# stemangiola/ppcseq

Hardware: AMD Instinct MI355X
Metric: effective samples/sec (whole node) for NB hierarchical fit (higher is better)
Workload: dtype f64; 1 GPU; BASELINE cfg3: synthetic 20000 genes x 200 samples (seed 20253), C=2, K=1000; NUTS (Stan defaults) warm-up 150 + 250 kept draws/chain, 8 chains per GPU (cfg3 names 8 chains; chains are the sharded unit, so N GPUs run 8N chains); mode=chains, chains_total=8, lanes_per_gene=4, loglik_workgroups=939, ess_estimator=rank-normalised split-chain bulk-ESS, min over 6 hyper-parameters and lp__, grad_evals=1471121, divergent_after_warmup=0, round_structure=pipelined: merged log-likelihood / state-machine launch + gene kernel, stream_groups=library default (3 from eight chains on, 2 from four), rounds_last_step_all_groups=115040

## Files before the change

ppcseq_amd/csrc/ppcx_gene.h:

```cpp
#pragma once
#include "ppcx_nuts.h"


namespace ppcx {

template <int CM>
struct GeneCtx {
  static constexpr int NCM = CM + 1;
  int gg, ncoord;
  bool active, has_slopes, fast, two;
  int idx[NCM];
  double q[NCM];
  GeneParams<CM> gp;
};

PPCX_HD void coord_consts(const Dims& d, const VecRef& v, int i, double q) {
  if (i >= d.off_sigma_raw && i < d.off_tail) {
    v.at(V_C0, i) = fast_exp(-q); v.at(V_C2, i) = q;
  } else if (i >= d.off_intercept && i < d.off_sigma_raw) {
    v.at(V_C0, i) = fast_exp(q);
    if (d.raw_consts) v.at(V_C2, i) = q;
  }
}

template <int CM>
PPCX_HD void gene_index(const Dims& d, int g, GeneCtx<CM>& x) {
  constexpr int NCM = CM + 1;
  x.active = g < d.G;
  x.gg = x.active ? g : 0;
  const int C = d.C;
  const int nslope = x.gg < d.K ? (C - 1 > 1 ? C - 1 : 1) : 0;
  x.ncoord = x.active ? 2 + nslope : 0;
#pragma unroll
  for (int j = 0; j < NCM; ++j)
    x.idx[j] = j == 0 ? d.off_intercept + x.gg : (j == 1 ? d.off_sigma_raw + x.gg : coef_index(d, j - 1, x.gg));
  x.has_slopes = x.active && x.gg < d.K && C >= 2;
  x.two = x.has_slopes && d.x0_is_one && d.x1_binary;
  x.fast = d.x0_is_one && (!x.has_slopes || x.two);
}
template <int CM>
PPCX_HD void gene_params(const Dims& d, const VecRef& v, GeneCtx<CM>& x) {
  x.gp.coef[0] = x.q[0];
#pragma unroll
  for (int cc = 1; cc < CM; ++cc) x.gp.coef[cc] = (x.has_slopes && cc < d.C) ? x.q[cc + 1] : 0.0;
  x.gp.sigma_raw = x.q[1];
  x.gp.phi = x.active ? v.at(V_C0, x.idx[1]) : 1.0;
  x.gp.invphi = 0.0;
}
template <int CM>
PPCX_HD void gene_load(const Dims& d, const Cmd& c, const VecRef& v, int g, GeneCtx<CM>& x) {
  constexpr int NCM = CM + 1;
  gene_index<CM>(d, g, x);
#pragma unroll
  for (int j = 0; j < NCM; ++j) x.q[j] = j < x.ncoord ? v.at(V_Q0 + 3 * c.dir, x.idx[j]) : 0.0;
  gene_params<CM>(d, v, x);
}

struct CellData {
  const int* counts;
  const double* disp;
  const unsigned char* gflags;
  const double* Sy;
  const double* ncell;
  double e_min, e_max;
};

struct GenePre { double phi, sigma, a0, Sy, n; int flags; };
PPCX_HD GenePre gene_pre_load(const Dims& d, const VecRef& v, const CellData& m, int g) {
  GenePre r;
  r.phi = v.at(V_C0, d.off_sigma_raw + g);
  r.sigma = v.at(V_C2, d.off_sigma_raw + g);
  r.a0 = v.at(V_C0, d.off_intercept + g);
  r.Sy = m.Sy[g]; r.n = m.ncell[g]; r.flags = m.gflags[g];
  return r;
}
template <int L> struct DispDeal {
  static constexpr int NL = L >= 8 ? 4 : (L >= 4 ? 2 : 1);
  static constexpr int CH = kDispStride / NL;
};

template <int CM, int L, int MODE, bool MASKED, bool WIN>
PPCX_HD void sweep_cells(int S, const int* row, const double* sE, const double* sX1, int sub, double A, double A1, double one,
                         const GeneParams<CM>& gp, const double* tab, CellAcc<CM>& acc, const double* ec = nullptr, int C = 2) {
  const int nmin = S / L;
  const int nlane = nmin + (sub < S - nmin * L ? 1 : 0);
  const int* p = row + sub;
  const double* q = sE + sub;
  const double* qx = sX1 + sub;
  int y0 = p[0], y1 = p[L], y2 = p[2 * L], y3 = p[3 * L];
  int k = 0;
#define PPCX_SWEEP_CELL(Y, E, XB, OFF, COND)                                                    \
  if ((COND) && (!MASKED || (Y) >= 0)) {                                                        \
    if (MODE == 1) { const double a1_ = (XB) != 0.0 ? A1 : A;                                   \
                     const double rho_ = WIN ? cell_eval_win<CM, true>(Y, E, a1_, one, gp, tab, acc) : cell_eval<CM, true>(Y, E, a1_, gp, tab, acc); \
                     acc.Tx[1] = fma(XB, rho_, acc.Tx[1]); }                                    \
    else if (MODE == 2) {                                                                       \
      double a_ = (XB) != 0.0 ? A1 : A; double xk_[CM];                                         \
      _Pragma("unroll") for (int cc = 2; cc < CM; ++cc) { xk_[cc] = cc < C ? qx[(cc - 1) * S + (OFF)] : 0.0; a_ = xk_[cc] != 0.0 ? a_ * ec[cc] : a_; } \
      const double rho_ = WIN ? cell_eval_win<CM, true>(Y, E, a_, one, gp, tab, acc) : cell_eval<CM, true>(Y, E, a_, gp, tab, acc); \
      acc.Tx[1] = fma(XB, rho_, acc.Tx[1]);                                                     \
      _Pragma("unroll") for (int cc = 2; cc < CM; ++cc) acc.Tx[cc] = fma(xk_[cc], rho_, acc.Tx[cc]); \
    }                                                                                           \
    else if (MODE == 3) {                                                                       \
      double t_ = (XB) * ec[1]; double xk_[CM];                                                 \
      _Pragma("unroll") for (int cc = 2; cc < CM; ++cc) { xk_[cc] = cc < C ? qx[(cc - 1) * S + (OFF)] : 0.0; t_ = fma(xk_[cc], ec[cc], t_); } \
      const double rho_ = cell_eval<CM, true>(Y, E, A * fast_exp(t_), gp, tab, acc);           \
      acc.Tx[1] = fma(XB, rho_, acc.Tx[1]);                                                     \
      _Pragma("unroll") for (int cc = 2; cc < CM; ++cc) acc.Tx[cc] = fma(xk_[cc], rho_, acc.Tx[cc]); \
    }                                                                                           \
    else if (WIN) (void)cell_eval_win<CM, false>(Y, E, A, one, gp, tab, acc);                   \
    else (void)cell_eval<CM, false>(Y, E, A, gp, tab, acc);                                     \
  }
  for (; k + 4 <= nmin; k += 4) {
    const double e0 = q[0], e1 = q[L], e2 = q[2 * L], e3 = q[3 * L];
    double x0 = 0.0, x1 = 0.0, x2 = 0.0, x3 = 0.0;
    if (MODE != 0) { x0 = qx[0]; x1 = qx[L]; x2 = qx[2 * L]; x3 = qx[3 * L]; }
    p += 4 * L; q += 4 * L; qx += 4 * L;
    const int n0 = p[0], n1 = p[L], n2 = p[2 * L], n3 = p[3 * L];
    if (MODE == 0 && !MASKED && WIN) {
      CellMidWin c0, c1, c2, c3;
      (void)cell_front_win<CM, false>(y0, e0, A, one, gp, tab, acc, c0);
      (void)cell_front_win<CM, false>(y1, e1, A, one, gp, tab, acc, c1);
      (void)cell_front_win<CM, false>(y2, e2, A, one, gp, tab, acc, c2);
      (void)cell_front_win<CM, false>(y3, e3, A, one, gp, tab, acc, c3);
#if defined(__HIP_DEVICE_COMPILE__)
      __builtin_amdgcn_sched_barrier(0);
#endif
      cell_back_win<CM>(c0, acc); cell_back_win<CM>(c1, acc); cell_back_win<CM>(c2, acc); cell_back_win<CM>(c3, acc);
    } else if (MODE == 0 && !MASKED) {
      CellMid c0, c1, c2, c3;
      (void)cell_front<CM, false>(y0, e0, A, gp, tab, acc, c0);
      (void)cell_front<CM, false>(y1, e1, A, gp, tab, acc, c1);
      (void)cell_front<CM, false>(y2, e2, A, gp, tab, acc, c2);
      (void)cell_front<CM, false>(y3, e3, A, gp, tab, acc, c3);
#if defined(__HIP_DEVICE_COMPILE__)
      __builtin_amdgcn_sched_barrier(0);
#endif
      cell_back<CM>(c0, acc); cell_back<CM>(c1, acc); cell_back<CM>(c2, acc); cell_back<CM>(c3, acc);
    } else {
      PPCX_SWEEP_CELL(y0, e0, x0, -4 * L, true)
      PPCX_SWEEP_CELL(y1, e1, x1, -3 * L, true)
      PPCX_SWEEP_CELL(y2, e2, x2, -2 * L, true)
      PPCX_SWEEP_CELL(y3, e3, x3, -L, true)
    }
    y0 = n0; y1 = n1; y2 = n2; y3 = n3;
  }
  if (k < nlane) {
    const double e0 = q[0], e1 = q[L], e2 = q[2 * L], e3 = q[3 * L];
    double x0 = 0.0, x1 = 0.0, x2 = 0.0, x3 = 0.0;
    if (MODE != 0) { x0 = qx[0]; x1 = qx[L]; x2 = qx[2 * L]; x3 = qx[3 * L]; }
    PPCX_SWEEP_CELL(y0, e0, x0, 0, true)
    PPCX_SWEEP_CELL(y1, e1, x1, L, k + 1 < nlane)
    PPCX_SWEEP_CELL(y2, e2, x2, 2 * L, k + 2 < nlane)
    PPCX_SWEEP_CELL(y3, e3, x3, 3 * L, k + 3 < nlane)
  }
#undef PPCX_SWEEP_CELL
}

template <int CM, int L>
PPCX_HD void generic_cells(const Dims& d, const Cmd& c, const VecRef& v, int g, bool has_slopes, const int* row,
                           const double* sExpo, const double* sX, int sub, GeneParams<CM>& gp, const double* tab,
                           CellAcc<CM>& acc) {
  const int S = d.S, C = d.C;
  gp.coef[0] = v.at(V_C2, d.off_intercept + g);
#pragma unroll
  for (int cc = 1; cc < CM; ++cc) gp.coef[cc] = (has_slopes && cc < C) ? v.at(V_C2, coef_index(d, cc, g)) : 0.0;
  (void)c;
  for (int s = sub; s < S; s += L) {
    const int y = row[s];
    if (y >= 0) {
      double t = sExpo[s] + gp.sigma_raw;
#pragma unroll
      for (int cc = 0; cc < CM; ++cc) if (cc < C) t += sX[cc * S + s] * gp.coef[cc];
      const double u = fast_exp(t);
      const double rho = cell_eval<CM, true>(y, u, 1.0, gp, tab, acc);
#pragma unroll
      for (int cc = 0; cc < CM; ++cc) if (cc < C) acc.Tx[cc] = fma(sX[cc * S + s], rho, acc.Tx[cc]);
    }
  }
}

template <int CM, int L, int GEN = 3>
PPCX_HD void lane_gene_sums(const Dims& d, const Cmd& c, const VecRef& v, const CellData& m, int g, const GenePre& pre, int sub,
                            const double* sE, const double* sExpo, const double* sX, const double* tab, const double* wtab,
                            GeneSumsV<CM>& o
#ifdef PPCX_TRACE
                            , unsigned long long* trace_stamps = nullptr
#endif
                            ) {
#if defined(PPCX_TRACE) && defined(__HIP_DEVICE_COMPILE__)
#define PPCX_GSTAMP(k) do { if (trace_stamps) trace_stamps[k] = __builtin_readcyclecounter(); } while (0)
#else
#define PPCX_GSTAMP(k) ((void)0)
#endif
  const int S = d.S;
  const bool has_slopes = g < d.K && d.C >= 2;
  const bool two = has_slopes && d.x0_is_one && d.x1_binary;
  const bool lin = (GEN & 1) && d.x0_is_one && has_slopes && !two;
  const bool generic = (GEN & 2) && !d.x0_is_one;
  GeneParams<CM> gp;
  gp.phi = pre.phi;
  const double sigma = pre.sigma;
  gp.sigma_raw = sigma;
  gp.invphi = fast_rcp(gp.phi);
  const double A = pre.a0 * gp.invphi;
  const bool masked = (pre.flags & 1) != 0;
  const int* row = m.counts + (long)g * S;
  constexpr int NL = DispDeal<L>::NL, CH = DispDeal<L>::CH;
  const DispRef dr = disp_ref(sigma);
  const int fn = L == 1 ? 0 : sub / NL, jch = L == 1 ? 0 : sub - fn * NL;
  const bool tab_lane = dr.in && (L == 1 || fn < 2);
  const double* pc = m.disp + (((long)g * kDispPanels + dr.panel) * 2 + (fn & 1)) * kDispStride + jch * CH;
  double cf[CH], cf2[L == 1 ? CH : 1];
#pragma unroll
  for (int k = 0; k < CH; ++k) cf[k] = 0.0;
  cf2[0] = 0.0;
  if (tab_lane) {
#pragma unroll
    for (int k = 0; k < CH; ++k) cf[k] = pc[k];
    if (L == 1) {
#pragma unroll
      for (int k = 0; k < CH; ++k) cf2[k] = pc[kDispStride + k];
    }
  }
  CellAcc<CM> acc; acc.zero();
  PPCX_GSTAMP(5);
  if (GEN & 2) {
    if (PPCX_WAVE_ANY(generic)) {
      if (generic) generic_cells<CM, L>(d, c, v, g, has_slopes, row, sExpo, sX, sub, gp, tab, acc);
    }
  }
  GeneWindow gw; gw.k = 0; gw.ok = false; gw.scale = 1.0;
  bool win = false;
  if (!(GEN & 2) || PPCX_WAVE_ANY(!generic)) {
    if (!generic) {
      const bool any_masked = PPCX_WAVE_ANY(masked);
#define PPCX_SWEEP(MODE, A_LO, A_HI, A_, A1_, X1_, ...)                                                                  \
      gw = gene_window(fma(m.e_min, A_LO, 1.0), fma(m.e_max, A_HI, 1.0));                                                 \
      win = !any_masked && PPCX_WAVE_ALL(gw.ok);                                                                          \
      if (any_masked) sweep_cells<CM, L, MODE, true, false>(S, row, sE, X1_, sub, A_, A1_, 1.0, gp, tab, acc, ##__VA_ARGS__);   \
      else if (win) sweep_cells<CM, L, MODE, false, true>(S, row, sE, X1_, sub, (A_) * gw.scale, (A1_) * gw.scale, gw.scale, gp, wtab, acc, ##__VA_ARGS__); \
      else sweep_cells<CM, L, MODE, false, false>(S, row, sE, X1_, sub, A_, A1_, 1.0, gp, tab, acc, ##__VA_ARGS__);
      if ((GEN & 1) && PPCX_WAVE_ANY(lin)) {
        double be[CM];
        be[0] = 0.0;
#pragma unroll
        for (int cc = 1; cc < CM; ++cc) be[cc] = (lin && cc < d.C) ? v.at(V_C2, coef_index(d, cc, g)) : 0.0;
        if (any_masked) sweep_cells<CM, L, 3, true, false>(S, row, sE, sX + S, sub, A, A, 1.0, gp, tab, acc, be, d.C);
        else sweep_cells<CM, L, 3, false, false>(S, row, sE, sX + S, sub, A, A, 1.0, gp, tab, acc, be, d.C);
      } else if (CM > 2 && d.C > 2 && PPCX_WAVE_ANY(two)) {
        double ec[CM];
        ec[0] = 1.0;
        double a_lo = A, a_hi = A;
#pragma unroll
        for (int cc = 1; cc < CM; ++cc) {
          ec[cc] = (two && cc < d.C) ? v.at(V_C0, coef_index(d, cc, g)) : 1.0;
          a_lo = ec[cc] < 1.0 ? a_lo * ec[cc] : a_lo; a_hi = ec[cc] > 1.0 ? a_hi * ec[cc] : a_hi;
        }
        const double A1 = A * ec[1];
        PPCX_SWEEP(2, a_lo, a_hi, A, A1, sX + S, ec, d.C)
      } else if (PPCX_WAVE_ANY(two)) {
        const double A1 = two ? A * v.at(V_C0, coef_index(d, 1, g)) : A;
        PPCX_SWEEP(1, (A1 < A ? A1 : A), (A1 > A ? A1 : A), A, A1, sX + S)
      } else {
        PPCX_SWEEP(0, A, A, A, A, sX)
      }
#undef PPCX_SWEEP
    }
  }
  PPCX_GSTAMP(6);
  if (!win) gw.scale = 1.0;
  cell_acc_close<CM>(gp, acc, gw.scale, &o);
  if ((GEN & 1) && lin) o.Tx[0] = o.Sr;
  if (win && sub == 0 && gw.k != 0) {
    const double kd = (double)gw.k;
    const double klog2 = fma(kd, 6.93147180369123816490e-01, kd * 1.90821492927058770002e-10);
    o.lik -= klog2 * fma(gp.phi, pre.n, pre.Sy);
    o.dph -= klog2 * pre.n;
  }
  if (tab_lane) {
    double hv = cf[CH - 1];
#pragma unroll
    for (int k = CH - 2; k >= 0; --k) hv = fma(hv, dr.x, cf[k]);
    if (NL > 1) {
      const double x3 = dr.x * dr.x * dr.x, xc = CH == 3 ? x3 : x3 * x3;
      double xp = (jch & 1) ? xc : 1.0;
      if (NL > 2) xp = (jch & 2) ? xp * (xc * xc) : xp;
      hv *= xp;
    }
    if (L == 1) {
      double h2 = cf2[CH - 1];
#pragma unroll
      for (int k = CH - 2; k >= 0; --k) h2 = fma(h2, dr.x, cf2[k]);
      o.lik += hv; o.dph += h2;
    } else if (fn == 0) o.lik += hv;
    else o.dph += hv;
  }
  if (PPCX_WAVE_ANY(!dr.in)) {
    PPCX_KEEP_BRANCH();
    if (!dr.in) {
      double F, D;
      disp_row_at(row, S, sub, L, sigma, &F, &D);
      o.lik += F; o.dph += D;
    }
  }
}

struct GeneData { double Sy, SyE, ncell, Lg1, SyX[kMaxC], SX[kMaxC]; };
// ... 306 lines not shown
```

ppcseq_amd/csrc/ppcx_kernels.hip:

```cpp
#include <hip/hip_runtime.h>
#include <hip/hip_ext.h>
#include "ppcx_gene.h"
#include "ppcx_kernels.h"

namespace ppcx {

typedef int __attribute__((may_alias)) word_t;
typedef double2 __attribute__((may_alias)) dpair_t;

#ifndef PPCX_LOGLIK_OCC
#define PPCX_LOGLIK_OCC 2
#endif
#ifndef PPCX_LOGLIK_OCC_FAST
#define PPCX_LOGLIK_OCC_FAST 4
#endif
__device__ __forceinline__ double wave_xor_add_rt(double v, int lane_xor_mask) {
  const int src = (int)((threadIdx.x ^ (unsigned)lane_xor_mask) & 63u) << 2;
  const int lo = __builtin_amdgcn_ds_bpermute(src, __double2loint(v));
  const int hi = __builtin_amdgcn_ds_bpermute(src, __double2hiint(v));
  return v + __hiloint2double(hi, lo);
}
template <int CTRL, int ROW_MASK>
__device__ __forceinline__ double dpp_take(double v) {
  const int lo = __builtin_amdgcn_update_dpp(0, __double2loint(v), CTRL, ROW_MASK, 0xf, true);
  const int hi = __builtin_amdgcn_update_dpp(0, __double2hiint(v), CTRL, ROW_MASK, 0xf, true);
  return __hiloint2double(hi, lo);
}
template <int L>
__device__ __forceinline__ double group_sum(double v) {
  if (L >= 2) v += dpp_take<0xB1, 0xf>(v);
  if (L >= 4) v += dpp_take<0x4E, 0xf>(v);
  if (L >= 8) v += dpp_take<0x141, 0xf>(v);
  if (L >= 16) v += dpp_take<0x140, 0xf>(v);
  if (L >= 32) v = wave_xor_add_rt(v, 16);
  if (L >= 64) v = wave_xor_add_rt(v, 32);
  return v;
}
template <int CM, int LG, int GEN>
__device__ __forceinline__ void loglik_passes(const LoglikArgs& a, const Cmd& c, const VecRef& v, double* sums, int p0, int p1,
                                              const double* stab, const double* swin, const double* sE, const double* sExpo, const double* sX,
                                              int lane, bool any_generic) {
  constexpr int L = 1 << LG, GPW = 64 >> LG;
  const Dims& d = a.d;
  const int sub = lane & (L - 1), gl = lane >> LG;
  int g_cur = a.order[p0 + gl < p1 ? p0 + gl : p1 - 1];
  int g_next = a.order[p0 + GPW + gl < p1 ? p0 + GPW + gl : p1 - 1];
  GenePre pre_cur = gene_pre_load(d, v, a.cd, g_cur);
#ifdef PPCX_TRACE
  unsigned long long* tr = nullptr;
  if (a.trace && lane == 0 && (blockIdx.x % 16) == 0 && blockIdx.x / 16 < kTraceBlocks)
    tr = a.trace + (((long)(blockIdx.x / 16) * 4 + (threadIdx.x >> 6)) * kTracePasses) * kTraceStamps;
  int tpass = 0;
#define PPCX_STAMP(k) do { if (tr && tpass < kTracePasses) tr[tpass * kTraceStamps + (k)] = __builtin_readcyclecounter(); } while (0)
#else
#define PPCX_STAMP(k) ((void)0)
#endif
  for (int p = p0; p < p1; p += GPW) {
    PPCX_STAMP(0);
#ifdef PPCX_TRACE
    if (tr && tpass < kTracePasses) tr[tpass * kTraceStamps + 7] = __builtin_amdgcn_s_memrealtime();
#endif
#ifdef PPCX_PRIO_BALANCE
    {
      const int rem = (p1 - p + GPW - 1) / GPW;
      if (rem >= 4) __builtin_amdgcn_s_setprio(3); else if (rem == 3) __builtin_amdgcn_s_setprio(2); else if (rem == 2) __builtin_amdgcn_s_setprio(1); else __builtin_amdgcn_s_setprio(0);
    }
#endif
    const bool act = p + gl < p1;
    const int g = g_cur;
    const GenePre pre = pre_cur;
    if (p + GPW < p1) {
      g_cur = g_next;
      pre_cur = gene_pre_load(d, v, a.cd, g_next);
      const int pn = p + 2 * GPW + gl;
      g_next = a.order[pn < p1 ? pn : p1 - 1];
    }
    if (CM > 2 && d.x0_is_one && !PPCX_WAVE_ANY(g < d.K)) {
      GeneSumsV<2> o2;
      lane_gene_sums<2, L, 0>(d, c, v, a.cd, g, pre, sub, sE, sExpo, sX, stab, swin, o2);
      o2.lik = group_sum<L>(o2.lik); o2.dph = group_sum<L>(o2.dph); o2.Sr = group_sum<L>(o2.Sr);
      if (act && sub == 0) { const long G = d.G; sums[0 * G + g] = o2.lik; sums[1 * G + g] = o2.dph; sums[2 * G + g] = o2.Sr; }
      continue;
    }
    GeneSumsV<CM> o;
    PPCX_STAMP(1);
#ifdef PPCX_TRACE
    lane_gene_sums<CM, L, GEN>(d, c, v, a.cd, g, pre, sub, sE, sExpo, sX, stab, swin, o, (tr && tpass < kTracePasses) ? tr + tpass * kTraceStamps : nullptr);
#else
    lane_gene_sums<CM, L, GEN>(d, c, v, a.cd, g, pre, sub, sE, sExpo, sX, stab, swin, o);
#endif
    PPCX_STAMP(2);
    const bool with_tx = any_generic && (!d.x0_is_one || PPCX_WAVE_ANY(g < d.K));
    o.lik = group_sum<L>(o.lik); o.dph = group_sum<L>(o.dph); o.Sr = group_sum<L>(o.Sr);
    PPCX_STAMP(3);
    if (with_tx) {
#pragma unroll
      for (int cc = 0; cc < CM; ++cc) if (cc < d.C) o.Tx[cc] = group_sum<L>(o.Tx[cc]);
    }
    if (act && sub == 0) {
      const long G = d.G;
      sums[0 * G + g] = o.lik; sums[1 * G + g] = o.dph; sums[2 * G + g] = o.Sr;
      if (with_tx) {
#pragma unroll
        for (int cc = 0; cc < CM; ++cc) if (cc < d.C) sums[(3 + cc) * G + g] = o.Tx[cc];
      }
    }
    PPCX_STAMP(4);
#ifdef PPCX_TRACE
    ++tpass;
#endif
  }
#undef PPCX_STAMP
}

template <int CM, int GEN, bool PIPE>
__device__ __forceinline__ void loglik_role(const LoglikArgs& a, int jb, int col, double* lds) {
  if (jb >= a.nbpc) return;
  constexpr int NS = GeneSums<CM>::N;
  const Dims& d = a.d;
  const int S = d.S, C = d.C;
  const int tid = threadIdx.x;
  const int wave = tid >> 6, lane = tid & 63;
  static_assert(2 * kLogTabSize == 2 * 256, "one 16-byte request per thread fills the table");
  const bool any_generic = !d.x0_is_one || (C >= 2 && d.K > 0);
  const bool evenS = (S & 1) == 0;
  const int p0 = a.bounds[jb * 4 + wave], p1 = a.bounds[jb * 4 + wave + 1];
  const double2 f_tab = reinterpret_cast<const dpair_t*>(a.logtab)[tid];
  static_assert(2 * kWinTabSize == 4 * 2 * 256, "four 16-byte requests per thread fill the window table");
  double2 f_win[4];
#pragma unroll
  for (int k = 0; k < 4; ++k) f_win[k] = reinterpret_cast<const dpair_t*>(a.wintab)[tid + 256 * k];
  double2 f_e = {0.0, 0.0};
  if (evenS) { if (tid < S / 2) f_e = reinterpret_cast<const dpair_t*>(a.sampleE)[tid]; }
  else if (tid < S) f_e.x = a.sampleE[tid];
  double f_x = 0.0;
  if (GEN != 2 && any_generic && tid < S) f_x = a.X[S + tid];
  const int chain = a.active ? a.active[col] : col;
  const Cmd& c = a.cmds[chain];
  if (c.type == CMD_DONE || c.type == CMD_FLUSH) return;
  if (PIPE) {
    if (c.evaluated && c.type != CMD_LEAF) return;
  }
  double* stab = lds;
  double* swin = lds + 2 * kLogTabSize;
  double* sE = swin + 2 * kWinTabSize;
  double* sExpo = GEN == 2 ? sE + S + kLdsPad : nullptr;
  double* sX = GEN == 2 ? sExpo + S : sE + kLdsPad;
  const VecRef v{a.vecs + (long)chain * V_COUNT * a.Dpad, a.Dpad};
  double* sums = a.sums + (long)chain * NS * d.G;
  reinterpret_cast<dpair_t*>(stab)[tid] = f_tab;
#pragma unroll
  for (int k = 0; k < 4; ++k) reinterpret_cast<dpair_t*>(swin)[tid + 256 * k] = f_win[k];
  if (evenS) {
    if (tid < S / 2) reinterpret_cast<dpair_t*>(sE)[tid] = f_e;
    for (int i = tid + 256; i < S / 2; i += 256) reinterpret_cast<dpair_t*>(sE)[i] = reinterpret_cast<const dpair_t*>(a.sampleE)[i];
  } else {
    if (tid < S) sE[tid] = f_e.x;
    for (int i = tid + 256; i < S; i += 256) sE[i] = a.sampleE[i];
  }
  if (any_generic) {
    if (GEN == 2) {
      for (int i = tid; i < S; i += 256) sExpo[i] = a.exposure[i];
      for (int i = tid; i < S * C; i += 256) sX[i] = a.X[i];
    } else {
      if (tid < S) sX[S + tid] = f_x;
      for (int i = tid + 256; i < S; i += 256) sX[S + i] = a.X[S + i];
      for (int i = 2 * S + tid; i < S * C; i += 256) sX[i] = a.X[i];
    }
  }
  __syncthreads();
  if (p0 >= p1) return;
  switch (a.lgL) {
    case 0: loglik_passes<CM, 0, GEN>(a, c, v, sums, p0, p1, stab, swin, sE, sExpo, sX, lane, any_generic); break;
    case 1: loglik_passes<CM, 1, GEN>(a, c, v, sums, p0, p1, stab, swin, sE, sExpo, sX, lane, any_generic); break;
    case 2: loglik_passes<CM, 2, GEN>(a, c, v, sums, p0, p1, stab, swin, sE, sExpo, sX, lane, any_generic); break;
    case 3: loglik_passes<CM, 3, GEN>(a, c, v, sums, p0, p1, stab, swin, sE, sExpo, sX, lane, any_generic); break;
    case 4: loglik_passes<CM, 4, GEN>(a, c, v, sums, p0, p1, stab, swin, sE, sExpo, sX, lane, any_generic); break;
    case 5: loglik_passes<CM, 5, GEN>(a, c, v, sums, p0, p1, stab, swin, sE, sExpo, sX, lane, any_generic); break;
    default: loglik_passes<CM, 6, GEN>(a, c, v, sums, p0, p1, stab, swin, sE, sExpo, sX, lane, any_generic); break;
  }
}

template <int CM, int GEN>
__global__ __launch_bounds__(256, GEN ? PPCX_LOGLIK_OCC : PPCX_LOGLIK_OCC_FAST) void ppcx_loglik_kernel(LoglikArgs a) {
  extern __shared__ double lds[];
  const int nch = a.nchains;
  const int lin = blockIdx.x, run = lin / (8 * nch), r = lin - run * (8 * nch);
  loglik_role<CM, GEN, false>(a, run * 8 + (r & 7), r >> 3, lds);
}

__device__ __forceinline__ double wave_sum_to_lane63(double v) {
  v += dpp_take<0x111, 0xf>(v);
  v += dpp_take<0x112, 0xf>(v);
  v += dpp_take<0x114, 0xf>(v);
  v += dpp_take<0x118, 0xf>(v);
  v += dpp_take<0x142, 0xa>(v);
  v += dpp_take<0x143, 0xc>(v);
  return v;
}
template <int N>
__device__ __forceinline__ void block_accumulate(double* vals, double* wacc, int wave, int lane) {
#pragma unroll
  for (int k = 0; k < N; ++k) vals[k] = wave_sum_to_lane63(vals[k]);
  if (lane == 63) {
#pragma unroll
    for (int k = 0; k < N; ++k) wacc[wave * PT_COUNT + k] = vals[k];
  }
}
struct ScanSums {
  static constexpr bool kLevel0WithLeaf = false;
  double* wacc; int wave, lane;
  __device__ __forceinline__ double* begin(int, double* own) {
#pragma unroll
    for (int k = 0; k < 6; ++k) own[k] = 0.0;
    return own;
  }
  __device__ __forceinline__ void end(int off, double* six) { block_accumulate<6>(six, wacc + off, wave, lane); }
};
__device__ __forceinline__ void slab_row_write(const Cmd& c, const double* wacc, double* slab, int tid, bool keep_t0) {
  const int np = parts_used(c);
  for (int k = tid; k < np; k += 256) {
    if (keep_t0 && k == PT_T0) continue;
    const bool used = k < 10 || (k >= PT_DOTS && k < PT_DOTS + 6 * c.n_merge) || (k >= PT_TOP && c.subtree_complete);
    slab[k] = used ? ((wacc[k] + wacc[PT_COUNT + k]) + wacc[2 * PT_COUNT + k]) + wacc[3 * PT_COUNT + k] : 0.0;
  }
}

constexpr int kRowStride = 65, kPartStride = 16, kRowsPerWave = 16;
template <int N>
__device__ __forceinline__ void wave_sums_lds(const double* vals, double* rows, double* out , int lane) {
  static_assert(N >= 1 && N <= kRowsPerWave, "one batch");
#pragma unroll
  for (int k = 0; k < N; ++k) rows[k * kRowStride + lane + (kPartStride - 16) * (lane >> 4)] = vals[k];
  __builtin_amdgcn_fence(__ATOMIC_RELEASE, "wavefront");
  __builtin_amdgcn_wave_barrier();
  const int k = lane >> 2, part = lane & 3;
  double t = 0.0;
  if (k < N) {
    const double* r = rows + k * kRowStride + kPartStride * part;
    double b[8];
#pragma unroll
    for (int j = 0; j < 8; ++j) b[j] = r[2 * j + 1] + r[2 * j];
    t = ((b[7] + b[6]) + (b[5] + b[4])) + ((b[3] + b[2]) + (b[1] + b[0]));
  }
  t += dpp_take<0xB1, 0xf>(t);
  t += dpp_take<0x4E, 0xf>(t);
  if (k < N && part == 0) out[k] = t;
  __builtin_amdgcn_fence(__ATOMIC_RELEASE, "wavefront");
  __builtin_amdgcn_wave_barrier();
}

template <int CM>
__global__ __launch_bounds__(256) void ppcx_close_kernel(CloseArgs a) {
  constexpr int NCM = CM + 1;
  constexpr int NS = GeneSums<CM>::N;
  __shared__ double wacc[4 * PT_COUNT];
  const int chain = blockIdx.y;
// ... 670 lines not shown
```

ppcseq_amd/csrc/ppcx_model.h:

```cpp
#pragma once
#include "ppcx_math.h"
#include "ppcx_disp.h"

namespace ppcx {

constexpr int kMaxC = 16;

struct Dims {
  int G, S, C, K, D;
  int off_intercept, off_alpha1, off_alpha2, off_sigma_raw, off_tail;
  int x0_is_one;
  int x1_binary;
  int raw_consts;
  int Gt, Kt, g0, k0;
  int gstride;
  double lambda_mu_mu;
};

PPCX_HD Dims make_dims(int G, int S, int C, int K, double lambda_mu_mu) {
  Dims d;
  d.G = G; d.S = S; d.C = C; d.K = K;
  d.off_intercept = 3;
  d.off_alpha1 = 3 + G;
  d.off_alpha2 = d.off_alpha1 + K;
  d.off_sigma_raw = d.off_alpha2 + (C > 2 ? C - 2 : 0) * K;
  d.off_tail = d.off_sigma_raw + G;
  d.D = d.off_tail + 3;
  d.x0_is_one = 1; d.x1_binary = 0; d.raw_consts = 0; d.lambda_mu_mu = lambda_mu_mu;
  d.Gt = G; d.Kt = K; d.g0 = 0; d.k0 = 0; d.gstride = 1;
  return d;
}
PPCX_HD int global_flat(const Dims& d, int i) {
  if (d.Gt == d.G) return i;
  const int n2 = d.C > 2 ? d.C - 2 : 0, st = d.gstride;
  if (i < d.off_intercept) return i;
  if (i < d.off_alpha1) return 3 + d.g0 + st * (i - d.off_intercept);
  if (i < d.off_alpha2) return 3 + d.Gt + d.k0 + st * (i - d.off_alpha1);
  if (i < d.off_sigma_raw) {
    const int j = i - d.off_alpha2, kl = j / n2, c = j - kl * n2;
    return 3 + d.Gt + d.Kt + n2 * (d.k0 + st * kl) + c;
  }
  const int sr_t = 3 + d.Gt + d.Kt + n2 * d.Kt;
  if (i < d.off_tail) return sr_t + d.g0 + st * (i - d.off_sigma_raw);
  return sr_t + d.Gt + (i - d.off_tail);
}
PPCX_HD int hyper_index(const Dims& d, int k) { return k < 3 ? k : d.off_tail + (k - 3); }
PPCX_HD int coef_index(const Dims& d, int c, int g) {
  return c == 0 ? d.off_intercept + g : (c == 1 ? d.off_alpha1 + g : d.off_alpha2 + (c - 2) + (d.C - 2) * g);
}

struct Hyper {
  double lambda_mu, lambda_sigma, lambda_skew, sigma_slope, sigma_intercept, sigma_sigma;
  double xi, inv_om, log_om, inv_ss, inv_ss2, log_ss;
};
PPCX_HD Hyper make_hyper(const double* u6, double lambda_mu_mu) {
  Hyper h;
  h.lambda_mu = u6[0] + lambda_mu_mu;
  h.lambda_sigma = fast_exp(u6[1]);
  h.lambda_skew = u6[2];
  h.sigma_slope = -fast_exp(u6[3]);
  h.sigma_intercept = u6[4];
  h.sigma_sigma = fast_exp(u6[5]);
  h.xi = h.lambda_mu + lambda_mu_mu;
  h.inv_om = fast_rcp(h.lambda_sigma); h.log_om = u6[1];
  h.inv_ss = fast_rcp(h.sigma_sigma); h.inv_ss2 = h.inv_ss * h.inv_ss; h.log_ss = u6[5];
  return h;
}

template <int CM>
struct GeneParams {
  double coef[CM];
  double sigma_raw, phi, invphi;
};

template <int CM>
struct CellAcc {
  double SA;
  double SL;
  double Sq;
  double SYq;
  double Tx[CM];
  PPCX_HD void zero() { SA = SL = Sq = SYq = 0.0;
#pragma unroll
    for (int c = 0; c < CM; ++c) Tx[c] = 0.0; }
};

#if defined(__HIP_DEVICE_COMPILE__)
#define PPCX_WAVE_ANY(p) (__any(p) != 0)
#define PPCX_WAVE_ALL(p) (__all(p) != 0)
#define PPCX_KEEP_BRANCH() asm volatile("" ::: "memory")
#define PPCX_OPAQUE(x) asm volatile("" : "+v"(x))
#else
#define PPCX_WAVE_ANY(p) (p)
#define PPCX_WAVE_ALL(p) (p)
#define PPCX_KEEP_BRANCH() ((void)0)
#define PPCX_OPAQUE(x) ((void)0)
#endif

struct CellMid { double yd, m, cinv, logc; int ex; };
template <int CM, bool SLOPES>
PPCX_HD double cell_front(int y, double e, double A, const GeneParams<CM>& gp, const double* tab, CellAcc<CM>& a, CellMid& c) {
#if defined(__HIP_DEVICE_COMPILE__) && !defined(PPCX_NO_ASM_CELL)
  double w, q, t;
  asm("v_cvt_f64_u32_e32 %[yd], %[y]\n\t"
      "v_fma_f64 %[w], %[e], %[A], 1.0\n\t"
      "v_rcp_f64_e32 %[q], %[w]\n\t"
      "v_frexp_mant_f64_e32 %[m], %[w]\n\t"
      "v_frexp_exp_i32_f64_e32 %[ex], %[w]\n\t"
      "v_fma_f64 %[t], -%[w], %[q], 1.0\n\t"
      "v_fma_f64 %[q], %[q], %[t], %[q]"
      : [yd] "=&v"(c.yd), [w] "=&v"(w), [q] "=&v"(q), [t] "=&v"(t), [m] "=&v"(c.m), [ex] "=&v"(c.ex)
      : [y] "v"(y), [e] "v"(e), [A] "v"(A));
#else
  c.yd = (double)y;
  const double w = fma(e, A, 1.0);
  const double q = fast_rcp(w);
  c.m = frexp(w, &c.ex);
#endif
  const int j = (int)(dbl_bits(w) >> (52 - kLogTabBits)) & (kLogTabSize - 1);
  c.cinv = tab[j]; c.logc = tab[kLogTabSize + j];
  a.Sq += q; a.SYq = fma(c.yd, q, a.SYq);
  return SLOPES ? fma(c.yd, gp.invphi, 1.0) * q : 0.0;
}
template <int CM>
PPCX_HD void cell_back(const CellMid& c, CellAcc<CM>& a) {
  double l;
#if defined(__HIP_DEVICE_COMPILE__) && !defined(PPCX_NO_ASM_CELL)
  double ed, r;
  const double L4 = -0.25;
  asm("v_fma_f64 %[r], %[m], %[cinv], -1.0\n\t"
      "v_cvt_f64_i32_e32 %[ed], %[ex]\n\t"
      "v_fma_f64 %[p], %[r], %[L5], %[L4]\n\t"
      "v_fma_f64 %[p], %[r], %[p], %[L3]\n\t"
      "v_fma_f64 %[p], %[r], %[p], -0.5\n\t"
      "v_fma_f64 %[p], %[r], %[p], 1.0\n\t"
      "v_fma_f64 %[p], %[r], %[p], %[logc]\n\t"
      "v_fma_f64 %[p], %[ed], %[LN2], %[p]"
      : [r] "=&v"(r), [ed] "=&v"(ed), [p] "=&v"(l)
      : [m] "v"(c.m), [ex] "v"(c.ex), [cinv] "v"(c.cinv), [logc] "v"(c.logc), [L4] "v"(L4),
        [L5] "s"(0.2), [L3] "s"(1.0 / 3.0), [LN2] "s"(6.93147180559945286227e-01));
#else
  const double r = fma(c.m, c.cinv, -1.0);
  double p = fma(r, 0.2, -0.25);
  p = fma(r, p, 1.0 / 3.0);
  p = fma(r, p, -0.5);
  p = fma(r, p, 1.0);
  l = fma((double)c.ex, 6.93147180559945286227e-01, fma(r, p, c.logc));
#endif
  a.SA = fma(c.yd, l, a.SA);
  a.SL += l;
}
template <int CM, bool SLOPES>
PPCX_HD double cell_eval(int y, double e, double A, const GeneParams<CM>& gp, const double* tab, CellAcc<CM>& a) {
  CellMid c;
  const double rho = cell_front<CM, SLOPES>(y, e, A, gp, tab, a, c);
  cell_back<CM>(c, a);
  return rho;
}

struct GeneWindow { int k; bool ok; double scale; };
PPCX_HD GeneWindow gene_window(double w_min, double w_max) {
  GeneWindow g;
  const int e0 = (int)((dbl_bits(w_min) >> 52) & 0x7ff), e1 = (int)((dbl_bits(w_max) >> 52) & 0x7ff);
  g.k = e0 - 1023;
  g.ok = w_min >= 1.0 && e1 - e0 < kWinBinades && e1 < 0x7ff;
  g.scale = bits_dbl((unsigned long long)(g.ok ? 2046 - e0 : 1023) << 52);
  if (!g.ok) g.k = 0;
  return g;
}
struct CellMidWin { double yd, w, cinv, logc; };
template <int CM, bool SLOPES>
PPCX_HD double cell_front_win(int y, double e, double A, double one, const GeneParams<CM>& gp, const double* wt, CellAcc<CM>& a, CellMidWin& c) {
  double q;
#if defined(__HIP_DEVICE_COMPILE__) && !defined(PPCX_NO_ASM_CELL)
  double t;
  asm("v_fma_f64 %[w], %[e], %[A], %[one]\n\t"
      "v_rcp_f64_e32 %[q], %[w]\n\t"
      "v_cvt_f64_u32_e32 %[yd], %[y]\n\t"
      "v_fma_f64 %[t], -%[w], %[q], 1.0\n\t"
      "v_fma_f64 %[q], %[q], %[t], %[q]"
      : [yd] "=&v"(c.yd), [w] "=&v"(c.w), [q] "=&v"(q), [t] "=&v"(t)
      : [y] "v"(y), [e] "v"(e), [A] "v"(A), [one] "v"(one));
#else
  c.yd = (double)y;
  c.w = fma(e, A, one);
  q = fast_rcp(c.w);
#endif
  const int j = (int)(dbl_bits(c.w) >> (52 - 8)) & (kWinTabSize - 1);
  const WinEntry we = window_entry(wt, j);
  c.cinv = we.cinv; c.logc = we.logc;
  a.Sq += q; a.SYq = fma(c.yd, q, a.SYq);
  return SLOPES ? fma(c.yd, gp.invphi, 1.0) * q : 0.0;
}
template <int CM>
PPCX_HD void cell_back_win(const CellMidWin& c, CellAcc<CM>& a) {
  double l;
#if defined(__HIP_DEVICE_COMPILE__) && !defined(PPCX_NO_ASM_CELL)
  double r;
  const double L4 = -0.25;
  asm("v_fma_f64 %[r], %[w], %[cinv], -1.0\n\t"
      "v_fma_f64 %[p], %[r], %[L5], %[L4]\n\t"
      "v_fma_f64 %[p], %[r], %[p], %[L3]\n\t"
      "v_fma_f64 %[p], %[r], %[p], -0.5\n\t"
      "v_fma_f64 %[p], %[r], %[p], 1.0\n\t"
      "v_fma_f64 %[p], %[r], %[p], %[logc]"
      : [r] "=&v"(r), [p] "=&v"(l)
      : [w] "v"(c.w), [cinv] "v"(c.cinv), [logc] "v"(c.logc), [L4] "v"(L4), [L5] "s"(0.2), [L3] "s"(1.0 / 3.0));
#else
  const double r = fma(c.w, c.cinv, -1.0);
  double p = fma(r, 0.2, -0.25);
  p = fma(r, p, 1.0 / 3.0);
  p = fma(r, p, -0.5);
  p = fma(r, p, 1.0);
  l = fma(r, p, c.logc);
#endif
  a.SA = fma(c.yd, l, a.SA);
  a.SL += l;
}
template <int CM, bool SLOPES>
PPCX_HD double cell_eval_win(int y, double e, double A, double one, const GeneParams<CM>& gp, const double* wt, CellAcc<CM>& a) {
  CellMidWin c;
  const double rho = cell_front_win<CM, SLOPES>(y, e, A, one, gp, wt, a, c);
  cell_back_win<CM>(c, a);
  return rho;
}

template <int CM>
struct GeneSumsV { double lik, dph, Sr, Tx[CM]; };
template <int CM> struct GeneSums { static constexpr int N = 3 + CM; };

template <int CM>
PPCX_HD void cell_acc_close(const GeneParams<CM>& gp, const CellAcc<CM>& a, double scale, GeneSumsV<CM>* o) {
  o->lik = -fma(gp.phi, a.SL, a.SA);
  o->dph = -a.SL;
  o->Sr = scale * fma(gp.invphi, a.SYq, a.Sq);
#pragma unroll
  for (int c = 0; c < CM; ++c) o->Tx[c] = scale * a.Tx[c];
}

template <int CM>
struct GeneOut {
  double lp;
  double g_coef[CM], g_sigma_raw;
  double h[6];
};

template <int CM>
PPCX_HD void gene_close(const Dims& d, const Hyper& hy, int g, bool has_slopes, const GeneParams<CM>& gp,
                        const GeneSumsV<CM>& a, double Sy, double SyE, const double* SyX , const double* SX ,
                        double ncell, double Lg1, GeneOut<CM>* o) {
  const double SQRT1_2 = 0.70710678118654752440, SQRT_2_OVER_PI = 0.79788456080286535588;
  double lik = (SyE - Sy) + (a.lik - Lg1);
#pragma unroll
  for (int c = 0; c < CM; ++c) {
    o->g_coef[c] = 0.0;
    if (c < d.C && (c == 0 || has_slopes)) {
      lik += gp.coef[c] * SyX[c];
      o->g_coef[c] = gp.phi * (a.Tx[c] - SX[c]);
    }
  }
  o->g_sigma_raw = gp.phi * ((a.Sr - ncell) - a.dph);
  const double icpt = gp.coef[0];
  const double z = (icpt - hy.xi) * hy.inv_om;
  double lerfc, ratio;
  log_erfc_and_ratio(-hy.lambda_skew * z * SQRT1_2, &lerfc, &ratio);
  ratio *= SQRT_2_OVER_PI;
  const double dz = -z + hy.lambda_skew * ratio;
  double lp = lik - hy.log_om - 0.5 * z * z + lerfc;
  o->g_coef[0] += dz * hy.inv_om;
  o->h[0] = -dz * hy.inv_om;
  o->h[1] = -hy.inv_om - dz * z * hy.inv_om;
  o->h[2] = z * ratio;
  const double r = gp.sigma_raw - (hy.sigma_slope * icpt + hy.sigma_intercept);
  const double rs = r * hy.inv_ss2;
  lp += -hy.log_ss - 0.5 * r * rs;
  o->g_sigma_raw += -rs;
  o->g_coef[0] += hy.sigma_slope * rs;
  o->h[3] = icpt * rs;
  o->h[4] = rs;
  o->h[5] = (-1.0 + r * rs) * hy.inv_ss;
  if (g < d.K) {
    if (d.C >= 2) {
      const double al = gp.coef[1];
      lp += -fabs(al);
      o->g_coef[1] += (al > 0.0) ? -1.0 : (al < 0.0 ? 1.0 : 0.0);
    }
#pragma unroll
    for (int c = 2; c < CM; ++c) if (c < d.C) {
      lp += -0.5 * gp.coef[c] * gp.coef[c] * (1.0 / 6.25);
      o->g_coef[c] += -gp.coef[c] * (1.0 / 6.25);
    }
  }
  o->lp = lp;
}

PPCX_HD double hyper_close(const Dims& d, const Hyper& hy, const double* u6, double lp_genes, const double* hsum,
                           double* g6) {
  double lp = lp_genes;
  lp += u6[1] + u6[3] + u6[5];
  const double dm = hy.lambda_mu - d.lambda_mu_mu;
  lp += -0.125 * dm * dm - 0.125 * hy.lambda_sigma * hy.lambda_sigma - 0.5 * hy.lambda_skew * hy.lambda_skew;
  lp += -0.125 * hy.sigma_intercept * hy.sigma_intercept - 0.125 * hy.sigma_slope * hy.sigma_slope
        - 0.125 * hy.sigma_sigma * hy.sigma_sigma;
  g6[0] = hsum[0] - 0.25 * dm;
  g6[1] = (hsum[1] - 0.25 * hy.lambda_sigma) * hy.lambda_sigma + 1.0;
  g6[2] = hsum[2] - hy.lambda_skew;
  g6[3] = (hsum[3] - 0.25 * hy.sigma_slope) * hy.sigma_slope + 1.0;
  g6[4] = hsum[4] - 0.25 * hy.sigma_intercept;
  g6[5] = (hsum[5] - 0.25 * hy.sigma_sigma) * hy.sigma_sigma + 1.0;
  return lp;
}

}
```

Before: 464.3 ESS/s.

## Tune gene cell sweep codegen with global/LDS address spaces and 8-cell unroll

Casts gene, order and sums pointers to the global address space with 32-bit unsigned offsets so the compiler can emit cheaper global loads and stores. The window table lookup becomes an LDS vector load with bitfield-extract addressing done in inline asm. The per-cell polynomial constant is hoisted and made opaque so it stays in one register. The cell sweep is unrolled to 8 cells per trip for CM<=2 with rotated prefetch of counts. These changes target instruction count and address arithmetic in the hot log-likelihood loop, at the cost of more register pressure and an assumption that the table pointer really lives in LDS.

```diff
diff --git a/ppcseq_amd/csrc/ppcx_gene.h b/ppcseq_amd/csrc/ppcx_gene.h
--- a/ppcseq_amd/csrc/ppcx_gene.h
+++ b/ppcseq_amd/csrc/ppcx_gene.h
@@ -66,12 +66,37 @@
 };
 
 struct GenePre { double phi, sigma, a0, Sy, n; int flags; };
+#if defined(__HIP_DEVICE_COMPILE__)
+#define PPCX_GLOBAL __attribute__((address_space(1)))
+#else
+#define PPCX_GLOBAL
+#endif
+template <class T>
+PPCX_HD PPCX_GLOBAL T* as_global(T* p) { return (PPCX_GLOBAL T*)p; }
+template <class T>
+PPCX_HD T ld32(const PPCX_GLOBAL T* base, int i) {
+#if defined(__HIP_DEVICE_COMPILE__)
+  return *(const PPCX_GLOBAL T*)((const PPCX_GLOBAL char*)base + (unsigned)i * (unsigned)sizeof(T));
+#else
+  return base[i];
+#endif
+}
+template <class T>
+PPCX_HD void st32(PPCX_GLOBAL T* base, int i, T x) {
+#if defined(__HIP_DEVICE_COMPILE__)
+  *(PPCX_GLOBAL T*)((PPCX_GLOBAL char*)base + (unsigned)i * (unsigned)sizeof(T)) = x;
+#else
+  base[i] = x;
+#endif
+}
 PPCX_HD GenePre gene_pre_load(const Dims& d, const VecRef& v, const CellData& m, int g) {
   GenePre r;
-  r.phi = v.at(V_C0, d.off_sigma_raw + g);
-  r.sigma = v.at(V_C2, d.off_sigma_raw + g);
-  r.a0 = v.at(V_C0, d.off_intercept + g);
-  r.Sy = m.Sy[g]; r.n = m.ncell[g]; r.flags = m.gflags[g];
+  const PPCX_GLOBAL double* c0 = as_global<const double>(&v.at(V_C0, 0));
+  const PPCX_GLOBAL double* c2 = as_global<const double>(&v.at(V_C2, 0));
+  r.phi = ld32(c0, d.off_sigma_raw + g);
+  r.sigma = ld32(c2, d.off_sigma_raw + g);
+  r.a0 = ld32(c0, d.off_intercept + g);
+  r.Sy = ld32(as_global(m.Sy), g); r.n = ld32(as_global(m.ncell), g); r.flags = ld32(as_global(m.gflags), g);
   return r;
 }
 template <int L> struct DispDeal {
@@ -84,66 +109,91 @@
                          const GeneParams<CM>& gp, const double* tab, CellAcc<CM>& acc, const double* ec = nullptr, int C = 2) {
   const int nmin = S / L;
   const int nlane = nmin + (sub < S - nmin * L ? 1 : 0);
-  const int* p = row + sub;
+  const PPCX_GLOBAL int* p = as_global(row + sub);
   const double* q = sE + sub;
   const double* qx = sX1 + sub;
   int y0 = p[0], y1 = p[L], y2 = p[2 * L], y3 = p[3 * L];
   int k = 0;
+  double L4 = kCellL4;
+  PPCX_OPAQUE(L4);
 #define PPCX_SWEEP_CELL(Y, E, XB, OFF, COND)                                                    \
   if ((COND) && (!MASKED || (Y) >= 0)) {                                                        \
     if (MODE == 1) { const double a1_ = (XB) != 0.0 ? A1 : A;                                   \
-                     const double rho_ = WIN ? cell_eval_win<CM, true>(Y, E, a1_, one, gp, tab, acc) : cell_eval<CM, true>(Y, E, a1_, gp, tab, acc); \
+                     const double rho_ = WIN ? cell_eval_win<CM, true>(Y, E, a1_, one, gp, tab, acc, L4) : cell_eval<CM, true>(Y, E, a1_, gp, tab, acc, L4); \
                      acc.Tx[1] = fma(XB, rho_, acc.Tx[1]); }                                    \
     else if (MODE == 2) {                                                                       \
       double a_ = (XB) != 0.0 ? A1 : A; double xk_[CM];                                         \
       _Pragma("unroll") for (int cc = 2; cc < CM; ++cc) { xk_[cc] = cc < C ? qx[(cc - 1) * S + (OFF)] : 0.0; a_ = xk_[cc] != 0.0 ? a_ * ec[cc] : a_; } \
-      const double rho_ = WIN ? cell_eval_win<CM, true>(Y, E, a_, one, gp, tab, acc) : cell_eval<CM, true>(Y, E, a_, gp, tab, acc); \
+      const double rho_ = WIN ? cell_eval_win<CM, true>(Y, E, a_, one, gp, tab, acc, L4) : cell_eval<CM, true>(Y, E, a_, gp, tab, acc, L4); \
       acc.Tx[1] = fma(XB, rho_, acc.Tx[1]);                                                     \
       _Pragma("unroll") for (int cc = 2; cc < CM; ++cc) acc.Tx[cc] = fma(xk_[cc], rho_, acc.Tx[cc]); \
     }                                                                                           \
     else if (MODE == 3) {                                                                       \
       double t_ = (XB) * ec[1]; double xk_[CM];                                                 \
       _Pragma("unroll") for (int cc = 2; cc < CM; ++cc) { xk_[cc] = cc < C ? qx[(cc - 1) * S + (OFF)] : 0.0; t_ = fma(xk_[cc], ec[cc], t_); } \
-      const double rho_ = cell_eval<CM, true>(Y, E, A * fast_exp(t_), gp, tab, acc);           \
+      const double rho_ = cell_eval<CM, true>(Y, E, A * fast_exp(t_), gp, tab, acc, L4);       \
       acc.Tx[1] = fma(XB, rho_, acc.Tx[1]);                                                     \
       _Pragma("unroll") for (int cc = 2; cc < CM; ++cc) acc.Tx[cc] = fma(xk_[cc], rho_, acc.Tx[cc]); \
     }                                                                                           \
-    else if (WIN) (void)cell_eval_win<CM, false>(Y, E, A, one, gp, tab, acc);                   \
-    else (void)cell_eval<CM, false>(Y, E, A, gp, tab, acc);                                     \
-  }
-  for (; k + 4 <= nmin; k += 4) {
-    const double e0 = q[0], e1 = q[L], e2 = q[2 * L], e3 = q[3 * L];
-    double x0 = 0.0, x1 = 0.0, x2 = 0.0, x3 = 0.0;
-    if (MODE != 0) { x0 = qx[0]; x1 = qx[L]; x2 = qx[2 * L]; x3 = qx[3 * L]; }
-    p += 4 * L; q += 4 * L; qx += 4 * L;
-    const int n0 = p[0], n1 = p[L], n2 = p[2 * L], n3 = p[3 * L];
-    if (MODE == 0 && !MASKED && WIN) {
-      CellMidWin c0, c1, c2, c3;
-      (void)cell_front_win<CM, false>(y0, e0, A, one, gp, tab, acc, c0);
-      (void)cell_front_win<CM, false>(y1, e1, A, one, gp, tab, acc, c1);
-      (void)cell_front_win<CM, false>(y2, e2, A, one, gp, tab, acc, c2);
-      (void)cell_front_win<CM, false>(y3, e3, A, one, gp, tab, acc, c3);
+    else if (WIN) (void)cell_eval_win<CM, false>(Y, E, A, one, gp, tab, acc, L4);               \
+    else (void)cell_eval<CM, false>(Y, E, A, gp, tab, acc, L4);                                 \
+  }
 #if defined(__HIP_DEVICE_COMPILE__)
-      __builtin_amdgcn_sched_barrier(0);
+#define PPCX_SWEEP_HALVES() __builtin_amdgcn_sched_barrier(0)
+#else
+#define PPCX_SWEEP_HALVES() ((void)0)
 #endif
-      cell_back_win<CM>(c0, acc); cell_back_win<CM>(c1, acc); cell_back_win<CM>(c2, acc); cell_back_win<CM>(c3, acc);
-    } else if (MODE == 0 && !MASKED) {
-      CellMid c0, c1, c2, c3;
-      (void)cell_front<CM, false>(y0, e0, A, gp, tab, acc, c0);
-      (void)cell_front<CM, false>(y1, e1, A, gp, tab, acc, c1);
-      (void)cell_front<CM, false>(y2, e2, A, gp, tab, acc, c2);
-      (void)cell_front<CM, false>(y3, e3, A, gp, tab, acc, c3);
-#if defined(__HIP_DEVICE_COMPILE__)
-      __builtin_amdgcn_sched_barrier(0);
-#endif
-      cell_back<CM>(c0, acc); cell_back<CM>(c1, acc); cell_back<CM>(c2, acc); cell_back<CM>(c3, acc);
-    } else {
-      PPCX_SWEEP_CELL(y0, e0, x0, -4 * L, true)
-      PPCX_SWEEP_CELL(y1, e1, x1, -3 * L, true)
-      PPCX_SWEEP_CELL(y2, e2, x2, -2 * L, true)
-      PPCX_SWEEP_CELL(y3, e3, x3, -L, true)
-    }
-    y0 = n0; y1 = n1; y2 = n2; y3 = n3;
+#define PPCX_SWEEP_TRIP(Y0, Y1, Y2, Y3, N0, N1, N2, N3, B)                                                                   \
+  {                                                                                                                          \
+    const double e0 = q[(B)], e1 = q[(B) + L], e2 = q[(B) + 2 * L], e3 = q[(B) + 3 * L];                                     \
+    double x0 = 0.0, x1 = 0.0, x2 = 0.0, x3 = 0.0;                                                                           \
+    if (MODE != 0) { x0 = qx[(B)]; x1 = qx[(B) + L]; x2 = qx[(B) + 2 * L]; x3 = qx[(B) + 3 * L]; }                           \
+    N0 = p[(B) + 4 * L]; N1 = p[(B) + 5 * L]; N2 = p[(B) + 6 * L]; N3 = p[(B) + 7 * L];                                      \
+    if (MODE == 0 && !MASKED && WIN) {                                                                                       \
+       \
+      CellMidWin c0, c1, c2, c3;                                                                                             \
+      (void)cell_front_win<CM, false>(Y0, e0, A, one, gp, tab, acc, c0);                                                     \
+      (void)cell_front_win<CM, false>(Y1, e1, A, one, gp, tab, acc, c1);                                                     \
+      (void)cell_front_win<CM, false>(Y2, e2, A, one, gp, tab, acc, c2);                                                     \
+      (void)cell_front_win<CM, false>(Y3, e3, A, one, gp, tab, acc, c3);                                                     \
+      PPCX_SWEEP_HALVES();                                                                                                   \
+      cell_back_win<CM>(c0, acc, L4); cell_back_win<CM>(c1, acc, L4); cell_back_win<CM>(c2, acc, L4); cell_back_win<CM>(c3, acc, L4); \
+    } else if (MODE == 0 && !MASKED) {                                                                                       \
+      CellMid c0, c1, c2, c3;                                                                                                \
+      (void)cell_front<CM, false>(Y0, e0, A, gp, tab, acc, c0);                                                              \
+      (void)cell_front<CM, false>(Y1, e1, A, gp, tab, acc, c1);                                                              \
+      (void)cell_front<CM, false>(Y2, e2, A, gp, tab, acc, c2);                                                              \
+      (void)cell_front<CM, false>(Y3, e3, A, gp, tab, acc, c3);                                                              \
+      PPCX_SWEEP_HALVES();                                                                                                   \
+      cell_back<CM>(c0, acc, L4); cell_back<CM>(c1, acc, L4); cell_back<CM>(c2, acc, L4); cell_back<CM>(c3, acc, L4);         \
+    } else {                                                                                                                 \
+      PPCX_SWEEP_CELL(Y0, e0, x0, (B), true)                                                                                 \
+      PPCX_SWEEP_CELL(Y1, e1, x1, (B) + L, true)                                                                             \
+      PPCX_SWEEP_CELL(Y2, e2, x2, (B) + 2 * L, true)                                                                         \
+      PPCX_SWEEP_CELL(Y3, e3, x3, (B) + 3 * L, true)                                                                         \
+    }                                                                                                                        \
+  }
+  if (CM <= 2) {
+    for (; k + 8 <= nmin; k += 8) {
+      int n0, n1, n2, n3;
+      PPCX_SWEEP_TRIP(y0, y1, y2, y3, n0, n1, n2, n3, 0)
+      PPCX_SWEEP_TRIP(n0, n1, n2, n3, y0, y1, y2, y3, 4 * L)
+      p += 8 * L; q += 8 * L; qx += 8 * L;
+    }
+    if (k + 4 <= nmin) {
+      int n0, n1, n2, n3;
+      PPCX_SWEEP_TRIP(y0, y1, y2, y3, n0, n1, n2, n3, 0)
+      p += 4 * L; q += 4 * L; qx += 4 * L;
+      y0 = n0; y1 = n1; y2 = n2; y3 = n3;
+      k += 4;
+    }
+  } else {
+    for (; k + 4 <= nmin; k += 4) {
+      int n0, n1, n2, n3;
+      PPCX_SWEEP_TRIP(y0, y1, y2, y3, n0, n1, n2, n3, 0)
+      p += 4 * L; q += 4 * L; qx += 4 * L;
+      y0 = n0; y1 = n1; y2 = n2; y3 = n3;
+    }
   }
   if (k < nlane) {
     const double e0 = q[0], e1 = q[L], e2 = q[2 * L], e3 = q[3 * L];
@@ -154,6 +204,8 @@
     PPCX_SWEEP_CELL(y2, e2, x2, 2 * L, k + 2 < nlane)
     PPCX_SWEEP_CELL(y3, e3, x3, 3 * L, k + 3 < nlane)
   }
+#undef PPCX_SWEEP_TRIP
+#undef PPCX_SWEEP_HALVES
 #undef PPCX_SWEEP_CELL
 }
 
diff --git a/ppcseq_amd/csrc/ppcx_kernels.hip b/ppcseq_amd/csrc/ppcx_kernels.hip
--- a/ppcseq_amd/csrc/ppcx_kernels.hip
+++ b/ppcseq_amd/csrc/ppcx_kernels.hip
@@ -43,8 +43,10 @@
   constexpr int L = 1 << LG, GPW = 64 >> LG;
   const Dims& d = a.d;
   const int sub = lane & (L - 1), gl = lane >> LG;
-  int g_cur = a.order[p0 + gl < p1 ? p0 + gl : p1 - 1];
-  int g_next = a.order[p0 + GPW + gl < p1 ? p0 + GPW + gl : p1 - 1];
+  const PPCX_GLOBAL int* order = as_global(a.order);
+  asm volatile("" : "+s"(order));
+  int g_cur = ld32(order, p0 + gl < p1 ? p0 + gl : p1 - 1);
+  int g_next = ld32(order, p0 + GPW + gl < p1 ? p0 + GPW + gl : p1 - 1);
   GenePre pre_cur = gene_pre_load(d, v, a.cd, g_cur);
 #ifdef PPCX_TRACE
   unsigned long long* tr = nullptr;
@@ -73,13 +75,13 @@
       g_cur = g_next;
       pre_cur = gene_pre_load(d, v, a.cd, g_next);
       const int pn = p + 2 * GPW + gl;
-      g_next = a.order[pn < p1 ? pn : p1 - 1];
+      g_next = ld32(order, pn < p1 ? pn : p1 - 1);
     }
     if (CM > 2 && d.x0_is_one && !PPCX_WAVE_ANY(g < d.K)) {
       GeneSumsV<2> o2;
       lane_gene_sums<2, L, 0>(d, c, v, a.cd, g, pre, sub, sE, sExpo, sX, stab, swin, o2);
       o2.lik = group_sum<L>(o2.lik); o2.dph = group_sum<L>(o2.dph); o2.Sr = group_sum<L>(o2.Sr);
-      if (act && sub == 0) { const long G = d.G; sums[0 * G + g] = o2.lik; sums[1 * G + g] = o2.dph; sums[2 * G + g] = o2.Sr; }
+      if (act && sub == 0) { const long G = d.G; st32(as_global(sums + 0 * G), g, o2.lik); st32(as_global(sums + 1 * G), g, o2.dph); st32(as_global(sums + 2 * G), g, o2.Sr); }
       continue;
     }
     GeneSumsV<CM> o;
@@ -99,10 +101,10 @@
     }
     if (act && sub == 0) {
       const long G = d.G;
-      sums[0 * G + g] = o.lik; sums[1 * G + g] = o.dph; sums[2 * G + g] = o.Sr;
+      st32(as_global(sums + 0 * G), g, o.lik); st32(as_global(sums + 1 * G), g, o.dph); st32(as_global(sums + 2 * G), g, o.Sr);
       if (with_tx) {
 #pragma unroll
-        for (int cc = 0; cc < CM; ++cc) if (cc < d.C) sums[(3 + cc) * G + g] = o.Tx[cc];
+        for (int cc = 0; cc < CM; ++cc) if (cc < d.C) st32(as_global(sums + (3 + cc) * G), g, o.Tx[cc]);
       }
     }
     PPCX_STAMP(4);
diff --git a/ppcseq_amd/csrc/ppcx_model.h b/ppcseq_amd/csrc/ppcx_model.h
--- a/ppcseq_amd/csrc/ppcx_model.h
+++ b/ppcseq_amd/csrc/ppcx_model.h
@@ -122,12 +122,12 @@
   a.Sq += q; a.SYq = fma(c.yd, q, a.SYq);
   return SLOPES ? fma(c.yd, gp.invphi, 1.0) * q : 0.0;
 }
-template <int CM>
-PPCX_HD void cell_back(const CellMid& c, CellAcc<CM>& a) {
+constexpr double kCellL4 = -0.25;
+template <int CM>
+PPCX_HD void cell_back(const CellMid& c, CellAcc<CM>& a, double L4 = kCellL4) {
   double l;
 #if defined(__HIP_DEVICE_COMPILE__) && !defined(PPCX_NO_ASM_CELL)
   double ed, r;
-  const double L4 = -0.25;
   asm("v_fma_f64 %[r], %[m], %[cinv], -1.0\n\t"
       "v_cvt_f64_i32_e32 %[ed], %[ex]\n\t"
       "v_fma_f64 %[p], %[r], %[L5], %[L4]\n\t"
@@ -146,15 +146,16 @@
   p = fma(r, p, -0.5);
   p = fma(r, p, 1.0);
   l = fma((double)c.ex, 6.93147180559945286227e-01, fma(r, p, c.logc));
+  (void)L4;
 #endif
   a.SA = fma(c.yd, l, a.SA);
   a.SL += l;
 }
 template <int CM, bool SLOPES>
-PPCX_HD double cell_eval(int y, double e, double A, const GeneParams<CM>& gp, const double* tab, CellAcc<CM>& a) {
+PPCX_HD double cell_eval(int y, double e, double A, const GeneParams<CM>& gp, const double* tab, CellAcc<CM>& a, double L4 = kCellL4) {
   CellMid c;
   const double rho = cell_front<CM, SLOPES>(y, e, A, gp, tab, a, c);
-  cell_back<CM>(c, a);
+  cell_back<CM>(c, a, L4);
   return rho;
 }
 
@@ -169,6 +170,19 @@
   return g;
 }
 struct CellMidWin { double yd, w, cinv, logc; };
+#if defined(__HIP_DEVICE_COMPILE__) && !defined(PPCX_NO_ASM_CELL)
+#define PPCX_LDS __attribute__((address_space(3)))
+__device__ __forceinline__ WinEntry window_entry_lds(const PPCX_LDS double* wt, double w) {
+  typedef double v2d_t __attribute__((ext_vector_type(2)));
+  const unsigned base = (unsigned)(unsigned long long)wt;
+  unsigned at;
+  asm("v_bfe_u32 %0, %1, 12, 10\n\t"
+      "v_lshl_add_u32 %0, %0, 4, %2"
+      : "=v"(at) : "v"(__double2hiint(w)), "s"(base));
+  const v2d_t e = *(const PPCX_LDS v2d_t*)at;
+  return WinEntry{e.x, e.y};
+}
+#endif
 template <int CM, bool SLOPES>
 PPCX_HD double cell_front_win(int y, double e, double A, double one, const GeneParams<CM>& gp, const double* wt, CellAcc<CM>& a, CellMidWin& c) {
   double q;
@@ -186,18 +200,21 @@
   c.w = fma(e, A, one);
   q = fast_rcp(c.w);
 #endif
+#if defined(__HIP_DEVICE_COMPILE__) && !defined(PPCX_NO_ASM_CELL)
+  const WinEntry we = window_entry_lds((const PPCX_LDS double*)wt, c.w);
+#else
   const int j = (int)(dbl_bits(c.w) >> (52 - 8)) & (kWinTabSize - 1);
   const WinEntry we = window_entry(wt, j);
+#endif
   c.cinv = we.cinv; c.logc = we.logc;
   a.Sq += q; a.SYq = fma(c.yd, q, a.SYq);
   return SLOPES ? fma(c.yd, gp.invphi, 1.0) * q : 0.0;
 }
 template <int CM>
-PPCX_HD void cell_back_win(const CellMidWin& c, CellAcc<CM>& a) {
+PPCX_HD void cell_back_win(const CellMidWin& c, CellAcc<CM>& a, double L4 = kCellL4) {
   double l;
 #if defined(__HIP_DEVICE_COMPILE__) && !defined(PPCX_NO_ASM_CELL)
   double r;
-  const double L4 = -0.25;
   asm("v_fma_f64 %[r], %[w], %[cinv], -1.0\n\t"
       "v_fma_f64 %[p], %[r], %[L5], %[L4]\n\t"
       "v_fma_f64 %[p], %[r], %[p], %[L3]\n\t"
@@ -213,15 +230,16 @@
   p = fma(r, p, -0.5);
   p = fma(r, p, 1.0);
   l = fma(r, p, c.logc);
+  (void)L4;
 #endif
   a.SA = fma(c.yd, l, a.SA);
   a.SL += l;
 }
 template <int CM, bool SLOPES>
-PPCX_HD double cell_eval_win(int y, double e, double A, double one, const GeneParams<CM>& gp, const double* wt, CellAcc<CM>& a) {
+PPCX_HD double cell_eval_win(int y, double e, double A, double one, const GeneParams<CM>& gp, const double* wt, CellAcc<CM>& a, double L4 = kCellL4) {
   CellMidWin c;
   const double rho = cell_front_win<CM, SLOPES>(y, e, A, one, gp, wt, a, c);
-  cell_back_win<CM>(c, a);
+  cell_back_win<CM>(c, a, L4);
   return rho;
 }
 
```

New measurement: 472.2 ESS/s (median of 6 runs). +1.7%, better.
